# hustvl/ControlAR

Hardware: AMD Instinct MI355X
Metric: images/sec/GPU, LlamaGen-XL t2i canny 512x512 (1024 tok); 1/2/4/8-GPU scaling (higher is better)
Workload: dtype bf16

## Files before the change

### controlar_amd/csrc/gemm.hip

```cpp
#include "car_common.h"
#include "gemm_gather.h"
#include <cstdio>
#include <cstdlib>

__device__ __forceinline__ void ld8bf(const bf16_t* p, float (&v)[8]) {
    const uint4 u = *(const uint4*)p; const unsigned w[4] = {u.x, u.y, u.z, u.w};
#pragma unroll
    for (int e = 0; e < 4; ++e) { v[2 * e] = __uint_as_float(w[e] << 16); v[2 * e + 1] = __uint_as_float(w[e] & 0xffff0000u); }
}
enum { EP_VEC = 0, EP_SCALAR = 1, EP_SWIGLU = 2 };
__device__ __forceinline__ float gate_act(int kind, float a) { return kind == 2 ? gelu_tanh_f(a) : silu_f(a); }
__device__ __forceinline__ int strip_path(const GemmP& p, long zC, long zR) {
    if (p.swiglu) return EP_SWIGLU;
    const bool vec = (p.N & 7) == 0 && (p.ldc & 7) == 0 && (!p.R || (p.ldr & 7) == 0) && p.bias_mode != BIAS_M &&
                     ((zC | zR) & 7) == 0 && ((uintptr_t)p.C & 15) == 0 && (!p.R || ((uintptr_t)p.R & 15) == 0);
    return vec ? EP_VEC : EP_SCALAR;
}
template <int PATH>
__device__ __forceinline__ void store_strip(const GemmP& p, const float* strip, int mb, int nb, long zC, long zR, int lane) {
    const bf16_t* bias = (const bf16_t*)p.bias; const bf16_t* scale = (const bf16_t*)p.scale; const bf16_t* R = (const bf16_t*)p.R;
    if (PATH == EP_SWIGLU) {
        const int rr = lane >> 2, c = (lane & 3) * 8, src = (c >> 4) * 32 + (c & 15), m = mb + rr;
        if (m < p.M && nb + src + 24 <= p.N && (p.ldc & 7) == 0 && (zC & 7) == 0) {
            unsigned o[4];
// ... 220 lines not shown
        if (kt + 2 < nk) issue(buf >= 1 ? buf - 1 : G2_NS - 1);
#pragma unroll
        for (int kk = 0; kk < 2; ++kk) {
            bf16x8 a[4], b[4];
#pragma unroll
            for (int i = 0; i < 4; ++i) { const int r = wm * 64 + i * 16 + fr; a[i] = *(const bf16x8*)(S2A(buf) + r * G2_BK + (((kk * 4 + fq) ^ (r & 7)) << 3)); }
#pragma unroll
            for (int j = 0; j < 4; ++j) { const int r = wn * 64 + j * 16 + fr; b[j] = *(const bf16x8*)(S2B(buf) + r * G2_BK + (((kk * 4 + fq) ^ (r & 7)) << 3)); }
#pragma unroll
            for (int i = 0; i < 4; ++i)
#pragma unroll
                for (int j = 0; j < 4; ++j)
                    acc[i][j] = __builtin_amdgcn_mfma_f32_16x16x32_bf16(a[i], b[j], acc[i][j], 0, 0, 0);
        }
        buf = buf + 1 == G2_NS ? 0 : buf + 1;
    }
    __syncthreads();

    float* strip = (float*)smem2 + wave * (16 * 68);
    const int path = strip_path(p, zC, zR);
#define STRIP_LOOP(PATH)                                                                          \
    _Pragma("unroll") for (int i = 0; i < 4; ++i) {                                               \
        _Pragma("unroll") for (int j = 0; j < 4; ++j) {                                           \
            const f32x4 q = acc[i][j];                                                            \
            float* d = strip + ((lane >> 4) * 4) * 68 + j * 16 + fr;                              \
            d[0] = q[0]; d[68] = q[1]; d[136] = q[2]; d[204] = q[3];                              \
        }                                                                                         \
        __builtin_amdgcn_wave_barrier();                                                          \
        store_strip<PATH>(p, strip, m0 + wm * 64 + i * 16, n0 + wn * 64, zC, zR, lane);           \
        __builtin_amdgcn_wave_barrier();                                                          \
    }
    if (path == EP_VEC) { STRIP_LOOP(EP_VEC) } else if (path == EP_SWIGLU) { STRIP_LOOP(EP_SWIGLU) } else { STRIP_LOOP(EP_SCALAR) }
#undef STRIP_LOOP
}

#define CH_HALO_MAX (18 * 18)
template <int UPS>
__global__ __launch_bounds__(512) void conv3_halo_kernel(GemmP p) {
    extern __shared__ __attribute__((aligned(16))) bf16_t smem3[];
    constexpr int HD = (16 >> UPS) + 2, HP = HD * HD;
    bf16_t* halo = smem3;
    bf16_t* wst = smem3 + CH_HALO_MAX * 128;
    const int tid = threadIdx.x, lane = tid & 63, wave = tid >> 6;
    const int wm = wave >> 1, wn = wave & 1;
    const int n0 = blockIdx.x * BN, tile = blockIdx.y;
    const int tw = p.Wo >> 4, th = p.Ho >> 4;
    const int b = tile / (tw * th), t2 = tile - b * (tw * th), ty = t2 / tw, tx = t2 - ty * tw;
    const int Hin = p.Ho >> UPS, Win = p.Wo >> UPS;
    const int hy0 = ((16 * ty - 1) >> UPS), hx0 = ((16 * tx - 1) >> UPS);
    const bf16_t* A = (const bf16_t*)p.A + (long)b * Hin * Win * p.Cin;
    const bf16_t* W = (const bf16_t*)p.W;
    const bf16_t* zero = (const bf16_t*)p.zero;
    const int fr = lane & 15, fq = lane >> 4;
    const int lr = lane >> 3, gchunk = ((lane & 7) ^ lr) * 8;
    const bf16_t* wrow[2];
#pragma unroll
    for (int i = 0; i < 2; ++i) { const int r = i * 64 + wave * 8 + lr; wrow[i] = (n0 + r) < p.N ? W + (long)(n0 + r) * p.ldw + gchunk : nullptr; }
    auto issue_w = [&](int buf, int kglob) {
#pragma unroll
        for (int i = 0; i < 2; ++i) {
            const bf16_t* src = wrow[i] ? wrow[i] + kglob : zero;
            __builtin_amdgcn_global_load_lds((gptr_t*)src, (lptr_t*)(wst + buf * (BN * G2_BK) + (i * 64 + wave * 8) * G2_BK), 16, 0, 0);
        }
    };
    f32x4 acc[4][4];
#pragma unroll
    for (int i = 0; i < 4; ++i)
#pragma unroll
        for (int j = 0; j < 4; ++j) acc[i][j] = (f32x4){0.f, 0.f, 0.f, 0.f};
    const int nchunk = p.Cin >> 7;
    for (int ch = 0; ch < nchunk; ++ch) {
        __syncthreads();
        for (int q = wave; q * 4 < HP; q += 8) {
            const int pix = q * 4 + (lane >> 4), slot = lane & 15;
            const int hy = pix / HD, hx = pix - hy * HD, iy = hy0 + hy, ix = hx0 + hx;
            const bf16_t* src = zero;
            if (pix < HP && iy >= 0 && iy < Hin && ix >= 0 && ix < Win) src = A + ((long)iy * Win + ix) * p.Cin + ch * 128 + ((slot ^ (pix & 15)) << 3);
            __builtin_amdgcn_global_load_lds((gptr_t*)src, (lptr_t*)(halo + q * 4 * 128), 16, 0, 0);
        }
        auto kglob = [&](int s_) { return (s_ >> 1) * p.Cin + ch * 128 + (s_ & 1) * 64; };
        issue_w(0, kglob(0)); issue_w(1, kglob(1));
        int buf = 0;
        for (int s_ = 0; s_ < 18; ++s_) {
            if (s_ == 0) asm volatile("s_waitcnt vmcnt(2)" ::: "memory");
            else if (s_ + 1 < 18) asm volatile("s_waitcnt vmcnt(2)" ::: "memory");
            else asm volatile("s_waitcnt vmcnt(0)" ::: "memory");
            __builtin_amdgcn_s_barrier();
            if (s_ + 2 < 18) issue_w(buf >= 1 ? buf - 1 : 2, kglob(s_ + 2));
            const int tap = s_ >> 1, c64 = s_ & 1, dy = tap / 3 - 1, dx = tap % 3 - 1;
            const bf16_t* ws = wst + buf * (BN * G2_BK);
#pragma unroll
            for (int kk = 0; kk < 2; ++kk) {
                bf16x8 a[4], bb[4];
#pragma unroll
                for (int i = 0; i < 4; ++i) {
                    const int h = (((16 * ty + wm * 4 + i + dy) >> UPS) - hy0) * HD + (((16 * tx + fr + dx) >> UPS) - hx0);
                    a[i] = *(const bf16x8*)(halo + h * 128 + (((c64 * 8 + kk * 4 + fq) ^ (h & 15)) << 3));
                }
#pragma unroll
                for (int j = 0; j < 4; ++j) { const int r = wn * 64 + j * 16 + fr; bb[j] = *(const bf16x8*)(ws + r * G2_BK + (((kk * 4 + fq) ^ (r & 7)) << 3)); }
#pragma unroll
                for (int i = 0; i < 4; ++i)
#pragma unroll
                    for (int j = 0; j < 4; ++j)
                        acc[i][j] = __builtin_amdgcn_mfma_f32_16x16x32_bf16(a[i], bb[j], acc[i][j], 0, 0, 0);
            }
            buf = buf + 1 == 3 ? 0 : buf + 1;
        }
    }
    __syncthreads();
    const bf16_t* bias = (const bf16_t*)p.bias; const bf16_t* R = (const bf16_t*)p.R;
    float* strip = (float*)smem3 + wave * (16 * 68);
    const int ec = (lane & 7) * 8, en = n0 + wn * 64 + ec;
    float bv[8];
    {
        const uint4 u = p.bias_mode == BIAS_N ? *(const uint4*)(bias + en) : make_uint4(0, 0, 0, 0);
        const unsigned w[4] = {u.x, u.y, u.z, u.w};
#pragma unroll
        for (int e = 0; e < 4; ++e) { bv[2 * e] = __uint_as_float(w[e] << 16); bv[2 * e + 1] = __uint_as_float(w[e] & 0xffff0000u); }
    }
#pragma unroll
    for (int i = 0; i < 4; ++i) {
#pragma unroll
        for (int j = 0; j < 4; ++j) {
            const f32x4 q = acc[i][j];
            float* d = strip + ((lane >> 4) * 4) * 68 + j * 16 + fr;
            d[0] = q[0]; d[68] = q[1]; d[136] = q[2]; d[204] = q[3];
        }
        __builtin_amdgcn_wave_barrier();
        const int oy = 16 * ty + wm * 4 + i;
#pragma unroll
        for (int pass = 0; pass < 2; ++pass) {
            const int rr = pass * 8 + (lane >> 3);
            const long mr = ((long)b * p.Ho + oy) * p.Wo + 16 * tx + rr;
            const float4 s0 = *(const float4*)(strip + rr * 68 + ec), s1 = *(const float4*)(strip + rr * 68 + ec + 4);
            float v[8] = {s0.x, s0.y, s0.z, s0.w, s1.x, s1.y, s1.z, s1.w};
#pragma unroll
            for (int e = 0; e < 8; ++e) v[e] = bf2f(f2bf(v[e] + bv[e]));
            if (R) {
                const uint4 u = *(const uint4*)(R + mr * p.ldr + en);
                const unsigned w[4] = {u.x, u.y, u.z, u.w};
#pragma unroll
                for (int e = 0; e < 4; ++e) { v[2 * e] = v[2 * e] + __uint_as_float(w[e] << 16); v[2 * e + 1] = v[2 * e + 1] + __uint_as_float(w[e] & 0xffff0000u); }
            }
            uint4 o;
            o.x = (unsigned)f2bf(v[0]) | ((unsigned)f2bf(v[1]) << 16); o.y = (unsigned)f2bf(v[2]) | ((unsigned)f2bf(v[3]) << 16);
            o.z = (unsigned)f2bf(v[4]) | ((unsigned)f2bf(v[5]) << 16); o.w = (unsigned)f2bf(v[6]) | ((unsigned)f2bf(v[7]) << 16);
            *(uint4*)((bf16_t*)p.C + mr * p.ldc + en) = o;
        }
        __builtin_amdgcn_wave_barrier();
    }
}

#define CH64_HALO_PIX 328
template <int UPS, int GNP>
__global__ __launch_bounds__(512, 4) void conv3_halo64_kernel(GemmP p) {
    extern __shared__ __attribute__((aligned(16))) bf16_t smem4[];
    constexpr int HD = (16 >> UPS) + 2, HP = HD * HD;
    bf16_t* halo = smem4;
    bf16_t* wst = smem4 + CH64_HALO_PIX * 64;
    const int tid = threadIdx.x, lane = tid & 63, wave = tid >> 6;
    const int wm = wave >> 1, wn = wave & 1;
    const int n0 = blockIdx.x * BN, tile = blockIdx.y;
    const int tw = p.Wo >> 4, th = p.Ho >> 4;
    const int b = tile / (tw * th), t2 = tile - b * (tw * th), ty = t2 / tw, tx = t2 - ty * tw;
    const int Hin = p.Ho >> UPS, Win = p.Wo >> UPS;
    const int hy0 = ((16 * ty - 1) >> UPS), hx0 = ((16 * tx - 1) >> UPS);
    const bf16_t* A = (const bf16_t*)p.A + (long)b * Hin * Win * p.Cin;
    const bf16_t* W = (const bf16_t*)p.W;
    const bf16_t* zero = (const bf16_t*)p.zero;
    const int fr = lane & 15, fq = lane >> 4;
    const int lr = lane >> 3, gchunk = ((lane & 7) ^ lr) * 8;
    const bf16_t* wrow[2];
#pragma unroll
    for (int i = 0; i < 2; ++i) { const int r = i * 64 + wave * 8 + lr; wrow[i] = (n0 + r) < p.N ? W + (long)(n0 + r) * p.ldw + gchunk : nullptr; }
    auto issue_w = [&](int buf, int kglob) {
#pragma unroll
        for (int i = 0; i < 2; ++i) {
            const bf16_t* src = wrow[i] ? wrow[i] + kglob : zero;
            __builtin_amdgcn_global_load_lds((gptr_t*)src, (lptr_t*)(wst + buf * (BN * G2_BK) + (i * 64 + wave * 8) * G2_BK), 16, 0, 0);
        }
    };
    f32x4 acc[4][4];
#pragma unroll
    for (int i = 0; i < 4; ++i)
#pragma unroll
        for (int j = 0; j < 4; ++j) acc[i][j] = (f32x4){0.f, 0.f, 0.f, 0.f};
    const int ngrp = p.Cin >> 6;
    for (int cg = 0; cg < ngrp; ++cg) {
        __syncthreads();
        for (int q = wave; q * 8 < HP; q += 8) {
            const int pix = q * 8 + (lane >> 3), slot = lane & 7;
            const int hy = pix / HD, hx = pix - hy * HD, iy = hy0 + hy, ix = hx0 + hx;
            const bf16_t* src = zero;
            if (pix < HP && iy >= 0 && iy < Hin && ix >= 0 && ix < Win) src = A + ((long)iy * Win + ix) * p.Cin + cg * 64 + ((slot ^ (pix & 7)) << 3);
            __builtin_amdgcn_global_load_lds((gptr_t*)src, (lptr_t*)(halo + q * 8 * 64), 16, 0, 0);
        }
        issue_w(0, cg * 64);
        int buf = 0;
        for (int tap = 0; tap < 9; ++tap) {
            asm volatile("s_waitcnt vmcnt(0)" ::: "memory");
            __builtin_amdgcn_s_barrier();
            if (tap + 1 < 9) issue_w(buf ^ 1, (tap + 1) * p.Cin + cg * 64);
            const int dy = tap / 3 - 1, dx = tap % 3 - 1;
            const bf16_t* ws = wst + buf * (BN * G2_BK);
#pragma unroll
            for (int kk = 0; kk < 2; ++kk) {
                bf16x8 a[4], bb[4];
#pragma unroll
                for (int i = 0; i < 4; ++i) {
                    const int h = (((16 * ty + wm * 4 + i + dy) >> UPS) - hy0) * HD + (((16 * tx + fr + dx) >> UPS) - hx0);
                    a[i] = *(const bf16x8*)(halo + h * 64 + (((kk * 4 + fq) ^ (h & 7)) << 3));
                }
#pragma unroll
                for (int j = 0; j < 4; ++j) { const int r = wn * 64 + j * 16 + fr; bb[j] = *(const bf16x8*)(ws + r * G2_BK + (((kk * 4 + fq) ^ (r & 7)) << 3)); }
#pragma unroll
                for (int i = 0; i < 4; ++i)
#pragma unroll
                    for (int j = 0; j < 4; ++j)
                        acc[i][j] = __builtin_amdgcn_mfma_f32_16x16x32_bf16(a[i], bb[j], acc[i][j], 0, 0, 0);
            }
            buf ^= 1;
        }
    }
    __syncthreads();
    const bf16_t* bias = (const bf16_t*)p.bias; const bf16_t* R = (const bf16_t*)p.R;
    float* strip = (float*)smem4 + wave * (16 * 68);
    const int ec = (lane & 7) * 8, en = n0 + wn * 64 + ec;
    float bv[8];
    {
        const uint4 u = p.bias_mode == BIAS_N ? *(const uint4*)(bias + en) : make_uint4(0, 0, 0, 0);
        const unsigned w[4] = {u.x, u.y, u.z, u.w};
#pragma unroll
        for (int e = 0; e < 4; ++e) { bv[2 * e] = __uint_as_float(w[e] << 16); bv[2 * e + 1] = __uint_as_float(w[e] & 0xffff0000u); }
    }
    float gs[8], gq[8];
#pragma unroll
    for (int e = 0; e < 8; ++e) { gs[e] = 0.f; gq[e] = 0.f; }
#pragma unroll
    for (int i = 0; i < 4; ++i) {
#pragma unroll
        for (int j = 0; j < 4; ++j) {
            const f32x4 q = acc[i][j];
            float* d = strip + ((lane >> 4) * 4) * 68 + j * 16 + fr;
            d[0] = q[0]; d[68] = q[1]; d[136] = q[2]; d[204] = q[3];
        }
        __builtin_amdgcn_wave_barrier();
        const int oy = 16 * ty + wm * 4 + i;
#pragma unroll
        for (int pass = 0; pass < 2; ++pass) {
            const int rr = pass * 8 + (lane >> 3);
            const long mr = ((long)b * p.Ho + oy) * p.Wo + 16 * tx + rr;
            const float4 s0 = *(const float4*)(strip + rr * 68 + ec), s1 = *(const float4*)(strip + rr * 68 + ec + 4);
            float v[8] = {s0.x, s0.y, s0.z, s0.w, s1.x, s1.y, s1.z, s1.w};
#pragma unroll
            for (int e = 0; e < 8; ++e) v[e] = bf2f(f2bf(v[e] + bv[e]));
            if (R) {
                const uint4 u = *(const uint4*)(R + mr * p.ldr + en);
                const unsigned w[4] = {u.x, u.y, u.z, u.w};
#pragma unroll
                for (int e = 0; e < 4; ++e) { v[2 * e] = v[2 * e] + __uint_as_float(w[e] << 16); v[2 * e + 1] = v[2 * e + 1] + __uint_as_float(w[e] & 0xffff0000u); }
            }
            uint4 o;
            o.x = (unsigned)f2bf(v[0]) | ((unsigned)f2bf(v[1]) << 16); o.y = (unsigned)f2bf(v[2]) | ((unsigned)f2bf(v[3]) << 16);
            o.z = (unsigned)f2bf(v[4]) | ((unsigned)f2bf(v[5]) << 16); o.w = (unsigned)f2bf(v[6]) | ((unsigned)f2bf(v[7]) << 16);
            *(uint4*)((bf16_t*)p.C + mr * p.ldc + en) = o;
            if (GNP) {
#pragma unroll
                for (int e = 0; e < 8; ++e) { const float r_ = bf2f(f2bf(v[e])); gs[e] += r_; gq[e] += r_ * r_; }
            }
        }
        __builtin_amdgcn_wave_barrier();
    }
    if (GNP) {
        float* red = (float*)smem4 + 8 * (16 * 68);
#pragma unroll
        for (int e = 0; e < 8; ++e) {
#pragma unroll
            for (int o_ = 8; o_ < 64; o_ <<= 1) { gs[e] += __shfl_xor(gs[e], o_, 64); gq[e] += __shfl_xor(gq[e], o_, 64); }
        }
        if (lane < 8) {
#pragma unroll
            for (int e = 0; e < 8; ++e) { red[(wave * 64 + lane * 8 + e) * 2] = gs[e]; red[(wave * 64 + lane * 8 + e) * 2 + 1] = gq[e]; }
        }
        __syncthreads();
        if (tid < 128) {
            const int wn2 = tid >> 6, cc = tid & 63;
            float s_ = 0.f, q_ = 0.f;
#pragma unroll
            for (int w4 = 0; w4 < 4; ++w4) { const float* r2 = red + ((w4 * 2 + wn2) * 64 + cc) * 2; s_ += r2[0]; q_ += r2[1]; }
            if (n0 + tid < p.N) {
                float* o2 = p.gn_part + ((long)b * (tw * th) + t2) * 2 * p.N;
                o2[n0 + tid] = s_; o2[p.N + n0 + tid] = q_;
            }
        }
    }
}

template <int AMODE>
__global__ __launch_bounds__(256) void gemm_f32_kernel(GemmP p) {
    __shared__ __attribute__((aligned(16))) float sA[2][16][68];
    __shared__ __attribute__((aligned(16))) float sB[2][16][68];
    const int tid = threadIdx.x, tx = tid & 15, ty = tid >> 4;
    const int z = blockIdx.z, z0 = z / p.nb1, z1 = z - z0 * p.nb1;
    const float* A = (const float*)p.A + z0 * p.sA0 + z1 * p.sA1;
    const float* W = (const float*)p.W + z0 * p.sW0 + z1 * p.sW1;
    const long zC = z0 * p.sC0 + z1 * p.sC1, zR = z0 * p.sR0 + z1 * p.sR1;
    const int m0 = blockIdx.y * 64, n0 = blockIdx.x * 64;
    const int lrow = tid >> 2, lkc = (tid & 3) * 4;
    const Geo geo = { p.M, p.Cin, p.Ho, p.Wo, p.ups, p.lda, p.patch };
    const ARow ar = make_arow<AMODE>(geo, m0 + lrow);
    const bool wok = (n0 + lrow) < p.N;
    const float* wp = W + (long)(n0 + lrow) * p.ldw + lkc;
    float4 ra, rb;
    const float4 zero4 = make_float4(0, 0, 0, 0);
    auto gload = [&](int kt) {
        long o = a_off<AMODE>(geo, ar, kt * 16 + lkc);
        ra = zero4; rb = zero4;
        if (o >= 0) ra = *(const float4*)(A + o);
        if (wok) rb = *(const float4*)(wp + (long)kt * 16);
    };
    auto sstore = [&](int buf) {
        sA[buf][lkc + 0][lrow] = ra.x; sA[buf][lkc + 1][lrow] = ra.y; sA[buf][lkc + 2][lrow] = ra.z; sA[buf][lkc + 3][lrow] = ra.w;
        sB[buf][lkc + 0][lrow] = rb.x; sB[buf][lkc + 1][lrow] = rb.y; sB[buf][lkc + 2][lrow] = rb.z; sB[buf][lkc + 3][lrow] = rb.w;
    };
    float acc[4][4] = {};
    const int nk = p.K / 16;
    gload(0); sstore(0);
    __syncthreads();
    for (int kt = 0; kt < nk; ++kt) {
        const int buf = kt & 1;
        if (kt + 1 < nk) gload(kt + 1);
#pragma unroll
        for (int k = 0; k < 16; ++k) {
            const float4 a = *(const float4*)&sA[buf][k][ty * 4];
            const float4 b = *(const float4*)&sB[buf][k][tx * 4];
            const float av[4] = {a.x, a.y, a.z, a.w}, bv[4] = {b.x, b.y, b.z, b.w};
#pragma unroll
            for (int i = 0; i < 4; ++i)
#pragma unroll
                for (int j = 0; j < 4; ++j) acc[i][j] = fmaf(av[i], bv[j], acc[i][j]);
        }
        if (kt + 1 < nk) sstore(buf ^ 1);
        __syncthreads();
    }
    const float* bias = (const float*)p.bias; const float* scale = (const float*)p.scale; const float* R = (const float*)p.R;
#pragma unroll
    for (int i = 0; i < 4; ++i)
#pragma unroll
        for (int j = 0; j < 4; ++j) {
            const int m = m0 + ty * 4 + i, n = n0 + tx * 4 + j;
            if (m < p.M && n < p.N)
                ((float*)p.C)[zC + (long)m * p.ldc + n] = epi_value<float>(p, bias, scale, R, zR, m, (long)m, n, acc[i][j]);
        }
}

typedef __attribute__((ext_vector_type(4))) float f4_t;
#define F32_LD 20
template <int AMODE>
__global__ __launch_bounds__(256) void gemm_f32_mfma_kernel(GemmP p) {
    __shared__ __attribute__((aligned(16))) float sA[2][128 * F32_LD];
    __shared__ __attribute__((aligned(16))) float sB[2][128 * F32_LD];
    const int tid = threadIdx.x, lane = tid & 63, wave = tid >> 6, q4 = lane >> 4, c16 = lane & 15;
    const int wm = wave >> 1, wn = wave & 1;
    const int z = blockIdx.z, z0 = z / p.nb1, z1 = z - z0 * p.nb1;
    const float* A = (const float*)p.A + z0 * p.sA0 + z1 * p.sA1;
    const float* W = (const float*)p.W + z0 * p.sW0 + z1 * p.sW1;
    const long zC = z0 * p.sC0 + z1 * p.sC1, zR = z0 * p.sR0 + z1 * p.sR1;
    const int m0 = blockIdx.y * 128, n0 = blockIdx.x * 128;
    const int lrow = tid >> 1, lkc = (tid & 1) * 8;
    const Geo geo = { p.M, p.Cin, p.Ho, p.Wo, p.ups, p.lda, p.patch };
    const ARow ar = make_arow<AMODE>(geo, m0 + lrow);
    const bool wok = (n0 + lrow) < p.N;
    const float* wp = W + (long)(n0 + lrow) * p.ldw + lkc;
    float4 ra[2], rb[2];
    const float4 zero4 = make_float4(0, 0, 0, 0);
    auto gload = [&](int kt) {
#pragma unroll
        for (int c = 0; c < 2; ++c) {
            const long o = a_off<AMODE>(geo, ar, kt * 16 + lkc + c * 4);
            ra[c] = zero4; rb[c] = zero4;
            if (o >= 0) ra[c] = *(const float4*)(A + o);
            if (wok) rb[c] = *(const float4*)(wp + (long)kt * 16 + c * 4);
        }
    };
    auto sstore = [&](int buf) {
#pragma unroll
        for (int c = 0; c < 2; ++c) { *(float4*)&sA[buf][lrow * F32_LD + lkc + c * 4] = ra[c]; *(float4*)&sB[buf][lrow * F32_LD + lkc + c * 4] = rb[c]; }
    };
    f4_t acc[4][4];
#pragma unroll
    for (int i = 0; i < 4; ++i)
#pragma unroll
        for (int j = 0; j < 4; ++j) acc[i][j] = (f4_t){0.f, 0.f, 0.f, 0.f};
    const int nk = p.K / 16;
    gload(0); sstore(0);
    __syncthreads();
    for (int kt = 0; kt < nk; ++kt) {
        const int buf = kt & 1;
        if (kt + 1 < nk) gload(kt + 1);
        f4_t xa[4], wa[4];
#pragma unroll
        for (int j = 0; j < 4; ++j) xa[j] = *(const f4_t*)&sA[buf][(wm * 64 + j * 16 + c16) * F32_LD + q4 * 4];
#pragma unroll
        for (int i = 0; i < 4; ++i) wa[i] = *(const f4_t*)&sB[buf][(wn * 64 + i * 16 + c16) * F32_LD + q4 * 4];
#pragma unroll
        for (int s = 0; s < 4; ++s)
#pragma unroll
            for (int i = 0; i < 4; ++i)
#pragma unroll
                for (int j = 0; j < 4; ++j) acc[i][j] = __builtin_amdgcn_mfma_f32_16x16x4f32(wa[i][s], xa[j][s], acc[i][j], 0, 0, 0);
        if (kt + 1 < nk) sstore(buf ^ 1);
        __syncthreads();
    }
    const float* bias = (const float*)p.bias; const float* scale = (const float*)p.scale; const float* R = (const float*)p.R;
    const bool vec = (p.ldc & 3) == 0 && ((zC & 3) == 0) && (((uintptr_t)p.C & 15) == 0);
#pragma unroll
    for (int j = 0; j < 4; ++j) {
        const int m = m0 + wm * 64 + j * 16 + c16;
        if (m >= p.M) continue;
#pragma unroll
        for (int i = 0; i < 4; ++i) {
            const int n = n0 + wn * 64 + i * 16 + q4 * 4;
            if (n >= p.N) continue;
            float v[4];
#pragma unroll
            for (int r = 0; r < 4; ++r) v[r] = (n + r < p.N) ? epi_value<float>(p, bias, scale, R, zR, m, (long)m, n + r, acc[i][j][r]) : 0.f;
            float* dst = (float*)p.C + zC + (long)m * p.ldc + n;
            if (vec && n + 3 < p.N) *(float4*)dst = make_float4(v[0], v[1], v[2], v[3]);
            else { for (int r = 0; r < 4; ++r) if (n + r < p.N) dst[r] = v[r]; }
        }
    }
}

static void* g_zero_page[16] = {};
static void* zero_page_for(int dev) {
    if (dev < 0 || dev >= 16) return nullptr;
    if (!g_zero_page[dev]) { if (hipMalloc(&g_zero_page[dev], 256) == hipSuccess) (void)hipMemset(g_zero_page[dev], 0, 256); else { g_zero_page[dev] = nullptr; (void)hipGetLastError(); } }
    return g_zero_page[dev];
}
static bool conv3_halo_plan(int mode, int amode, const GemmP& p, int* dev_out, void** zero_out) {
    int dev = 0; (void)hipGetDevice(&dev);
    if (dev_out) *dev_out = dev;
    if (!(mode == 1 && amode == AMODE_CONV3 && p.Cin % 128 == 0 && (p.Ho & 15) == 0 && (p.Wo & 15) == 0 && (p.ups == 0 || p.ups == 1) && p.K == 9 * p.Cin && p.ldw % 8 == 0 &&
          (uintptr_t)p.A % 16 == 0 && (uintptr_t)p.W % 16 == 0 && !p.swiglu && !p.out_f32 && p.act == ACT_NONE && (p.nb0 <= 1) && (p.nb1 <= 1) && p.alpha == 1.0f &&
          p.N % 128 == 0 && !p.scale && p.bias_mode != BIAS_M && p.ldc % 8 == 0 && (!p.R || p.ldr % 8 == 0) && !CAR_KNOB("CAR_GEMM_V1") && !CAR_KNOB("CAR_NO_HALO"))) return false;
    void* z = zero_page_for(dev);
    if (zero_out) *zero_out = z;
    return z != nullptr;
}
extern "C" int car_conv3_halo64_ok(int mode, const GemmP* pp) {
    return conv3_halo_plan(mode, AMODE_CONV3, *pp, nullptr, nullptr) && !CAR_KNOB("CAR_CONV_HALO128") && !CAR_KNOB("CAR_GN_UNFUSED");
}
extern "C" int car_gemm_split_ok(int amode, const GemmP* pp);
extern "C" hipError_t car_launch_gemm_split(int amode, const GemmP* pp, hipStream_t st);
extern "C" int car_gemm_route(int mode, int amode, const GemmP* pp) {
    const GemmP& p = *pp;
    const int nb0 = p.nb0 <= 0 ? 1 : p.nb0, nb1 = p.nb1 <= 0 ? 1 : p.nb1;
    if (mode == 1) {
        if (conv3_halo_plan(mode, amode, p, nullptr, nullptr)) {
            const bool halo128 = CAR_KNOB("CAR_CONV_HALO128") != nullptr;
            if (p.gn_part && (halo128 || CAR_KNOB("CAR_GN_UNFUSED"))) return CAR_ROUTE_REFUSE_GN;
            return halo128 ? CAR_ROUTE_HALO128 : CAR_ROUTE_HALO64;
        }
        if (p.gn_part) return CAR_ROUTE_REFUSE_GN;
        if (p.K % BKK != 0) return CAR_ROUTE_REFUSE_K;
        const bool al16 = ((uintptr_t)p.A % 16 == 0) && ((uintptr_t)p.W % 16 == 0) && p.ldw % 8 == 0 && p.sW0 % 8 == 0 && p.sW1 % 8 == 0 && p.sA0 % 8 == 0 && p.sA1 % 8 == 0;
        const long tiles = (long)((p.N + BN - 1) / BN) * ((p.M + G2_BM - 1) / G2_BM) * nb0 * nb1;
        int dev = 0; (void)hipGetDevice(&dev);
        const bool ok2 = dev >= 0 && dev < 16 && p.K % G2_BK == 0 && p.K >= 512 && al16 && tiles >= 512 && !CAR_KNOB("CAR_GEMM_V1") &&
                         (amode == AMODE_PLAIN ? p.lda % 8 == 0 : (amode == AMODE_CONV3 && p.Cin % G2_BK == 0));
        return ok2 ? CAR_ROUTE_BF16_GLDS : CAR_ROUTE_BF16_REG;
    }
    if (p.gn_part) return CAR_ROUTE_REFUSE_GN;
    if (p.K % 16 != 0) return CAR_ROUTE_REFUSE_K;
    if (p.split3 && car_gemm_split_ok(amode, &p)) return CAR_ROUTE_F32_SPLIT;
    const bool mfma_ok = p.ldw % 4 == 0 && ((uintptr_t)p.A & 15) == 0 && ((uintptr_t)p.W & 15) == 0 && p.sA0 % 4 == 0 && p.sA1 % 4 == 0 && p.sW0 % 4 == 0 && p.sW1 % 4 == 0 &&
                         (amode == AMODE_PLAIN ? p.lda % 4 == 0 : p.Cin % 4 == 0);
    return mfma_ok ? CAR_ROUTE_F32_MFMA : CAR_ROUTE_F32_VALU;
}
extern "C" int car_launch_gemm(int mode, int amode, const GemmP* pp, hipStream_t st) {
    GemmP p = *pp;
    if (p.nb0 <= 0) p.nb0 = 1;
    if (p.nb1 <= 0) p.nb1 = 1;
    const int route = car_gemm_route(mode, amode, &p);
    if (route < 0) {
        if (route == CAR_ROUTE_REFUSE_K) fprintf(stderr, "car_launch_gemm: K = %d is not a multiple of %d (%s kernels): refused, nothing launched\n", p.K, mode == 1 ? BKK : 16, mode == 1 ? "bf16" : "fp32");
        return route;
    }
    static bool attr_set[16] = {}, attr3[16] = {}, attr4[16] = {};
    int dev = 0; (void)hipGetDevice(&dev);
    if (mode == 1) { if (amode != AMODE_CONV3 || (p.Ho & 15) || (p.Wo & 15) || CAR_KNOB("CAR_CONV_LINEAR")) p.patch = 0; }
    else p.patch = 0;
    switch (route) {
    case CAR_ROUTE_HALO64: {
        p.zero = zero_page_for(dev);
        const dim3 g3((p.N + BN - 1) / BN, (unsigned)((long)p.M / 256));
        const size_t sh4 = (size_t)(CH64_HALO_PIX * 64 + 2 * BN * G2_BK) * 2;
        if (!attr4[dev]) {
            (void)hipFuncSetAttribute((const void*)conv3_halo64_kernel<0, 0>, hipFuncAttributeMaxDynamicSharedMemorySize, (int)sh4);
            (void)hipFuncSetAttribute((const void*)conv3_halo64_kernel<1, 0>, hipFuncAttributeMaxDynamicSharedMemorySize, (int)sh4);
            (void)hipFuncSetAttribute((const void*)conv3_halo64_kernel<0, 1>, hipFuncAttributeMaxDynamicSharedMemorySize, (int)sh4);
            (void)hipFuncSetAttribute((const void*)conv3_halo64_kernel<1, 1>, hipFuncAttributeMaxDynamicSharedMemorySize, (int)sh4);
            attr4[dev] = true;
        }
        if (p.ups == 0) { if (p.gn_part) hipLaunchKernelGGL((conv3_halo64_kernel<0, 1>), g3, dim3(512), sh4, st, p); else hipLaunchKernelGGL((conv3_halo64_kernel<0, 0>), g3, dim3(512), sh4, st, p); }
        else { if (p.gn_part) hipLaunchKernelGGL((conv3_halo64_kernel<1, 1>), g3, dim3(512), sh4, st, p); else hipLaunchKernelGGL((conv3_halo64_kernel<1, 0>), g3, dim3(512), sh4, st, p); }
        return 0;
    }
    case CAR_ROUTE_HALO128: {
        p.zero = zero_page_for(dev);
        const dim3 g3((p.N + BN - 1) / BN, (unsigned)((long)p.M / 256));
        const size_t sh3 = (size_t)(CH_HALO_MAX * 128 + 3 * BN * G2_BK) * 2;
        if (!attr3[dev]) {
            (void)hipFuncSetAttribute((const void*)conv3_halo_kernel<0>, hipFuncAttributeMaxDynamicSharedMemorySize, (int)sh3);
            (void)hipFuncSetAttribute((const void*)conv3_halo_kernel<1>, hipFuncAttributeMaxDynamicSharedMemorySize, (int)sh3);
            attr3[dev] = true;
        }
        if (p.ups == 0) hipLaunchKernelGGL(conv3_halo_kernel<0>, g3, dim3(512), sh3, st, p);
        else hipLaunchKernelGGL(conv3_halo_kernel<1>, g3, dim3(512), sh3, st, p);
        return 0;
    }
    case CAR_ROUTE_BF16_GLDS: {
        const size_t sh = (size_t)G2_NS * G2_STAGE * 2;
        if (!attr_set[dev]) {
            (void)hipFuncSetAttribute((const void*)gemm_bf16_glds_kernel<AMODE_PLAIN>, hipFuncAttributeMaxDynamicSharedMemorySize, (int)sh);
            (void)hipFuncSetAttribute((const void*)gemm_bf16_glds_kernel<AMODE_CONV3>, hipFuncAttributeMaxDynamicSharedMemorySize, (int)sh);
            attr_set[dev] = true;
        }
        if ((p.zero = zero_page_for(dev)) != nullptr) {
            dim3 g2((p.N + BN - 1) / BN, (p.M + G2_BM - 1) / G2_BM, p.nb0 * p.nb1);
            if (amode == AMODE_PLAIN) hipLaunchKernelGGL(gemm_bf16_glds_kernel<AMODE_PLAIN>, g2, dim3(512), sh, st, p);
            else hipLaunchKernelGGL(gemm_bf16_glds_kernel<AMODE_CONV3>, g2, dim3(512), sh, st, p);
            return 0;
        }
        [[fallthrough]];
    }
    case CAR_ROUTE_BF16_REG: {
        dim3 g((p.N + BN - 1) / BN, (p.M + BM - 1) / BM, p.nb0 * p.nb1);
        if (amode == AMODE_PLAIN) hipLaunchKernelGGL(gemm_bf16_kernel<AMODE_PLAIN>, g, dim3(256), 0, st, p);
        else if (amode == AMODE_CONV3S2) hipLaunchKernelGGL(gemm_bf16_kernel<AMODE_CONV3S2>, g, dim3(256), 0, st, p);
        else hipLaunchKernelGGL(gemm_bf16_kernel<AMODE_CONV3>, g, dim3(256), 0, st, p);
        return 0;
    }
    case CAR_ROUTE_F32_SPLIT:
        return car_launch_gemm_split(amode, &p, st) == hipSuccess ? 0 : -2;
    case CAR_ROUTE_F32_MFMA: {
        dim3 g((p.N + 127) / 128, (p.M + 127) / 128, p.nb0 * p.nb1);
        if (amode == AMODE_PLAIN) hipLaunchKernelGGL(gemm_f32_mfma_kernel<AMODE_PLAIN>, g, dim3(256), 0, st, p);
        else if (amode == AMODE_CONV3S2) hipLaunchKernelGGL(gemm_f32_mfma_kernel<AMODE_CONV3S2>, g, dim3(256), 0, st, p);
        else hipLaunchKernelGGL(gemm_f32_mfma_kernel<AMODE_CONV3>, g, dim3(256), 0, st, p);
        return 0;
    }
    default: {
        dim3 g((p.N + 63) / 64, (p.M + 63) / 64, p.nb0 * p.nb1);
        if (amode == AMODE_PLAIN) hipLaunchKernelGGL(gemm_f32_kernel<AMODE_PLAIN>, g, dim3(256), 0, st, p);
        else if (amode == AMODE_CONV3S2) hipLaunchKernelGGL(gemm_f32_kernel<AMODE_CONV3S2>, g, dim3(256), 0, st, p);
        else hipLaunchKernelGGL(gemm_f32_kernel<AMODE_CONV3>, g, dim3(256), 0, st, p);
        return 0;
    }
    }
}
```

Measured before the change: 44.85.

## Fully unroll halo64 conv tap loop with hand-scheduled LDS reads and waits

Adds a new default path in the 64-channel halo conv kernel. It unrolls all 9 taps at compile time, uses precomputed LDS byte offsets with inline ds_read_b128 immediates, and staggers the A/B fragment loads with fine-grained lgkmcnt waits and sched barriers so LDS reads overlap the MFMAs. The halo swizzle now uses the column index, which lets the address math be hoisted out of the loop, and the wave index is made uniform via readfirstlane. The old loop stays available behind a knob, and a bit-exact A/B check harness is added. The hand-written waitcnt logic and schedule are fragile and could raise register pressure at 4 waves per SIMD.

```diff
diff --git a/controlar_amd/csrc/gemm.hip b/controlar_amd/csrc/gemm.hip
--- a/controlar_amd/csrc/gemm.hip
+++ b/controlar_amd/csrc/gemm.hip
@@ -396,14 +396,27 @@
     }
 }
 
+template <int I> struct car_ic { static constexpr int value = I; };
+template <int N, int I = 0, class F> __device__ __forceinline__ void car_static_for(F&& f) { if constexpr (I < N) { f(car_ic<I>{}); car_static_for<N, I + 1>(f); } }
+template <int UPS> constexpr int h64_a_off(int tap, int g) { const int i = g & 3, dy = tap / 3 - 1; return (UPS ? (i + dy + 2) >> 1 : i + dy + 1) * ((16 >> UPS) + 2) * 128; }
+constexpr int h64_b_off(int buf, int j) { return buf * (BN * G2_BK * 2) + j * (16 * G2_BK * 2); }
+template <int OFF> __device__ __forceinline__ void lds_read16(bf16x8& v, unsigned addr) { asm volatile("ds_read_b128 %0, %1 offset:%2" : "=v"(v) : "v"(addr), "n"(OFF) : "memory"); }
+template <int N> __device__ __forceinline__ void lds_wait(bf16x8& x0) { asm volatile("s_waitcnt lgkmcnt(%1)" : "+v"(x0) : "n"(N)); }
+template <int N> __device__ __forceinline__ void lds_wait(bf16x8& x0, bf16x8& x1) { asm volatile("s_waitcnt lgkmcnt(%2)" : "+v"(x0), "+v"(x1) : "n"(N)); }
+template <int N> __device__ __forceinline__ void lds_wait(bf16x8& x0, bf16x8& x1, bf16x8& x2) { asm volatile("s_waitcnt lgkmcnt(%3)" : "+v"(x0), "+v"(x1), "+v"(x2) : "n"(N)); }
+template <int N> __device__ __forceinline__ void lds_wait(bf16x8& x0, bf16x8& x1, bf16x8& x2, bf16x8& x3, bf16x8& x4, bf16x8& x5) {
+    asm volatile("s_waitcnt lgkmcnt(%6)" : "+v"(x0), "+v"(x1), "+v"(x2), "+v"(x3), "+v"(x4), "+v"(x5) : "n"(N));
+}
 #define CH64_HALO_PIX 328
-template <int UPS, int GNP>
+template <int UPS, int GNP, int V1>
 __global__ __launch_bounds__(512, 4) void conv3_halo64_kernel(GemmP p) {
     extern __shared__ __attribute__((aligned(16))) bf16_t smem4[];
     constexpr int HD = (16 >> UPS) + 2, HP = HD * HD;
     bf16_t* halo = smem4;
     bf16_t* wst = smem4 + CH64_HALO_PIX * 64;
-    const int tid = threadIdx.x, lane = tid & 63, wave = tid >> 6;
+    const int tid = threadIdx.x, lane = tid & 63;
+    const int wave = V1 ? tid >> 6 : __builtin_amdgcn_readfirstlane(tid >> 6);
+
     const int wm = wave >> 1, wn = wave & 1;
     const int n0 = blockIdx.x * BN, tile = blockIdx.y;
     const int tw = p.Wo >> 4, th = p.Ho >> 4;
@@ -430,6 +443,10 @@
     for (int i = 0; i < 4; ++i)
 #pragma unroll
         for (int j = 0; j < 4; ++j) acc[i][j] = (f32x4){0.f, 0.f, 0.f, 0.f};
+    unsigned ho[3];
+#pragma unroll
+    for (int d = 0; d < 3; ++d) { const int col = UPS ? (fr + d + 1) >> 1 : fr + d; ho[d] = (unsigned)((wm * (4 >> UPS) * HD + col) * 128 + ((fq ^ (col & 7)) << 4)); }
+    const unsigned wo = (unsigned)(CH64_HALO_PIX * 128 + (wn * 64 + fr) * 128 + ((fq ^ (fr & 7)) << 4));
     const int ngrp = p.Cin >> 6;
     for (int cg = 0; cg < ngrp; ++cg) {
         __syncthreads();
@@ -437,10 +454,45 @@
             const int pix = q * 8 + (lane >> 3), slot = lane & 7;
             const int hy = pix / HD, hx = pix - hy * HD, iy = hy0 + hy, ix = hx0 + hx;
             const bf16_t* src = zero;
-            if (pix < HP && iy >= 0 && iy < Hin && ix >= 0 && ix < Win) src = A + ((long)iy * Win + ix) * p.Cin + cg * 64 + ((slot ^ (pix & 7)) << 3);
+            if (pix < HP && iy >= 0 && iy < Hin && ix >= 0 && ix < Win) src = A + ((long)iy * Win + ix) * p.Cin + cg * 64 + ((slot ^ ((V1 ? pix : hx) & 7)) << 3);
             __builtin_amdgcn_global_load_lds((gptr_t*)src, (lptr_t*)(halo + q * 8 * 64), 16, 0, 0);
         }
         issue_w(0, cg * 64);
+        if constexpr (!V1) {
+            bf16x8 a[3], b0[4], b1[4];
+            car_static_for<9>([&](auto tap_) {
+                constexpr int tap = decltype(tap_)::value, buf = tap & 1, last = tap == 8;
+                asm volatile("s_waitcnt vmcnt(0)" ::: "memory");
+                __builtin_amdgcn_s_barrier();
+                if (tap + 1 < 9) issue_w(buf ^ 1, (tap + 1) * p.Cin + cg * 64);
+                if (tap == 0) { lds_read16<h64_a_off<UPS>(0, 0)>(a[0], ho[0]); lds_read16<h64_a_off<UPS>(0, 1)>(a[1], ho[0]); }
+                car_static_for<4>([&](auto j_) { constexpr int j = decltype(j_)::value; lds_read16<h64_b_off(buf, j)>(b0[j], wo); });
+                car_static_for<8>([&](auto g_) {
+                    constexpr int g = decltype(g_)::value, G = tap * 8 + g, i = g & 3, c = G % 3, n2 = (G + 2) % 3;
+                    if constexpr (g + 2 < 8) lds_read16<h64_a_off<UPS>(tap, g + 2)>(a[n2], ho[tap % 3] ^ (unsigned)(((g + 2) >> 2) << 6));
+                    else if constexpr (!last) lds_read16<h64_a_off<UPS>(tap + 1, g - 6)>(a[n2], ho[(tap + 1) % 3]);
+                    if constexpr (g == 1) lds_read16<h64_b_off(buf, 0)>(b1[0], wo ^ 64u);
+                    if constexpr (g == 2) lds_read16<h64_b_off(buf, 1)>(b1[1], wo ^ 64u);
+                    if constexpr (g == 0) lds_wait<1>(a[c], a[(G + 1) % 3], b0[0], b0[1], b0[2], b0[3]);
+                    if constexpr (g == 2 || g == 3) lds_wait<4>(a[c]);
+                    if constexpr (g == 4) lds_wait<4>(a[c], b1[0], b1[1]);
+                    if constexpr (g == 6) lds_wait<last ? 1 : 2>(a[c]);
+                    if constexpr (g == 7) lds_wait<last ? 0 : 2>(a[c]);
+                    car_static_for<4>([&](auto j_) {
+                        constexpr int j = decltype(j_)::value;
+                        if constexpr (g == 4 && j == 2) { __builtin_amdgcn_sched_barrier(0); lds_wait<2>(a[(G + 1) % 3], b1[2]); }
+                        if constexpr (g == 4 && j == 3) { __builtin_amdgcn_sched_barrier(0); lds_wait<1>(b1[3]); }
+                        acc[i][j] = __builtin_amdgcn_mfma_f32_16x16x32_bf16(a[c], g < 4 ? b0[j] : b1[j], acc[i][j], 0, 0, 0);
+                        if constexpr (g == 3 && j < 2) {
+                            __builtin_amdgcn_sched_barrier(0);
+                            lds_read16<h64_b_off(buf, 2 + j)>(b1[2 + j], wo ^ 64u);
+                        }
+                    });
+                    __builtin_amdgcn_sched_barrier(0);
+                });
+            });
+            continue;
+        }
         int buf = 0;
         for (int tap = 0; tap < 9; ++tap) {
             asm volatile("s_waitcnt vmcnt(0)" ::: "memory");
@@ -741,15 +793,15 @@
         p.zero = zero_page_for(dev);
         const dim3 g3((p.N + BN - 1) / BN, (unsigned)((long)p.M / 256));
         const size_t sh4 = (size_t)(CH64_HALO_PIX * 64 + 2 * BN * G2_BK) * 2;
+        typedef void (*halo64_fn)(GemmP);
+        static const halo64_fn fn4[2][2][2] = {{{conv3_halo64_kernel<0, 0, 0>, conv3_halo64_kernel<0, 1, 0>}, {conv3_halo64_kernel<1, 0, 0>, conv3_halo64_kernel<1, 1, 0>}},
+                                               {{conv3_halo64_kernel<0, 0, 1>, conv3_halo64_kernel<0, 1, 1>}, {conv3_halo64_kernel<1, 0, 1>, conv3_halo64_kernel<1, 1, 1>}}};
         if (!attr4[dev]) {
-            (void)hipFuncSetAttribute((const void*)conv3_halo64_kernel<0, 0>, hipFuncAttributeMaxDynamicSharedMemorySize, (int)sh4);
-            (void)hipFuncSetAttribute((const void*)conv3_halo64_kernel<1, 0>, hipFuncAttributeMaxDynamicSharedMemorySize, (int)sh4);
-            (void)hipFuncSetAttribute((const void*)conv3_halo64_kernel<0, 1>, hipFuncAttributeMaxDynamicSharedMemorySize, (int)sh4);
-            (void)hipFuncSetAttribute((const void*)conv3_halo64_kernel<1, 1>, hipFuncAttributeMaxDynamicSharedMemorySize, (int)sh4);
+            for (int i = 0; i < 8; ++i) (void)hipFuncSetAttribute((const void*)fn4[i >> 2][(i >> 1) & 1][i & 1], hipFuncAttributeMaxDynamicSharedMemorySize, (int)sh4);
             attr4[dev] = true;
         }
-        if (p.ups == 0) { if (p.gn_part) hipLaunchKernelGGL((conv3_halo64_kernel<0, 1>), g3, dim3(512), sh4, st, p); else hipLaunchKernelGGL((conv3_halo64_kernel<0, 0>), g3, dim3(512), sh4, st, p); }
-        else { if (p.gn_part) hipLaunchKernelGGL((conv3_halo64_kernel<1, 1>), g3, dim3(512), sh4, st, p); else hipLaunchKernelGGL((conv3_halo64_kernel<1, 0>), g3, dim3(512), sh4, st, p); }
+        const int v1 = CAR_KNOB("CAR_CONV_TAPLOOP_V1") != nullptr;
+        hipLaunchKernelGGL(fn4[v1][p.ups][p.gn_part != nullptr], g3, dim3(512), sh4, st, p);
         return 0;
     }
     case CAR_ROUTE_HALO128: {
diff --git a/experiments/conv_pipe_check.hip b/experiments/conv_pipe_check.hip
--- /dev/null
+++ b/experiments/conv_pipe_check.hip
@@ -0,0 +1,186 @@
+#ifndef CAR_DEV_KNOBS
+#error "conv_pipe_check needs -DCAR_DEV_KNOBS: without it CAR_KNOB() is a null constant, CAR_CONV_TAPLOOP_V1 selects nothing and the new loop would be compared with itself"
+#endif
+#include "../controlar_amd/csrc/gemm.hip"
+#include "../controlar_amd/csrc/gemm_split.hip"
+#include "../controlar_amd/csrc/ops.hip"
+
+#include <cmath>
+#include <cstdio>
+#include <cstdlib>
+#include <cstring>
+#include <vector>
+
+extern "C" { int g_car_knob_hits = 0; }
+
+#define CK(x) do { hipError_t e_ = (x); if (e_ != hipSuccess) { printf("HIP error %s at %s:%d\n", hipGetErrorString(e_), __FILE__, __LINE__); exit(2); } } while (0)
+static const char* const SWITCH = "CAR_CONV_TAPLOOP_V1";
+static const size_t GUARD = 512;
+static int g_fail = 0;
+
+static unsigned hsh(unsigned a, unsigned b, unsigned seed) {
+    unsigned x = a * 2654435761u + b * 0x85ebca6bu + seed * 0x9e3779b9u; x ^= x >> 15; x *= 2246822519u; x ^= x >> 13; x *= 3266489917u; x ^= x >> 16; return x;
+}
+static bf16_t rnd_bf16(unsigned i, unsigned seed, unsigned expo) { const unsigned x = hsh(i, 0u, seed); return (bf16_t)((x & 0x807fu) | ((((x >> 7) & 3u) + expo) << 7)); }
+
+struct Case { const char* name; int B, Ho, Wo, Cin, Cout, ups; bool bias, resid, gn; };
+
+struct Bufs {
+    bf16_t *x = nullptr, *w = nullptr, *bias = nullptr, *r = nullptr, *y = nullptr; float* part = nullptr;
+    size_t nin = 0, nw = 0, nout = 0, npart = 0;
+};
+static void alloc(const Case& c, Bufs& d) {
+    const int Hin = c.Ho >> c.ups, Win = c.Wo >> c.ups;
+    d.nin = (size_t)c.B * Hin * Win * c.Cin; d.nw = (size_t)c.Cout * 9 * c.Cin; d.nout = (size_t)c.B * c.Ho * c.Wo * c.Cout;
+    d.npart = (size_t)c.B * (c.Ho / 16) * (c.Wo / 16) * 2 * c.Cout;
+    CK(hipMalloc(&d.x, d.nin * 2)); CK(hipMalloc(&d.w, d.nw * 2)); CK(hipMalloc(&d.bias, (size_t)c.Cout * 2)); CK(hipMalloc(&d.r, d.nout * 2));
+    CK(hipMalloc(&d.y, (d.nout + 2 * GUARD) * 2)); CK(hipMalloc(&d.part, (d.npart + 2 * GUARD) * 4));
+}
+static void release(Bufs& d) { for (void* q : {(void*)d.x, (void*)d.w, (void*)d.bias, (void*)d.r, (void*)d.y, (void*)d.part}) CK(hipFree(q)); }
+static void up(bf16_t* dst, const std::vector<bf16_t>& h) { CK(hipMemcpy(dst, h.data(), h.size() * 2, hipMemcpyHostToDevice)); }
+
+static void launch(const Case& c, const Bufs& d, bool v1, std::vector<unsigned char>& out, std::vector<unsigned char>& part) {
+    CK(hipMemset(d.y, 0xff, (d.nout + 2 * GUARD) * 2)); CK(hipMemset(d.part, 0xff, (d.npart + 2 * GUARD) * 4));
+    GemmP p; memset(&p, 0, sizeof(p));
+    p.A = d.x; p.W = d.w; p.C = d.y + GUARD; p.ldw = 9L * c.Cin; p.ldc = c.Cout; p.M = c.B * c.Ho * c.Wo; p.N = c.Cout; p.K = 9 * c.Cin; p.alpha = 1.f; p.nb0 = p.nb1 = 1;
+    p.Ho = c.Ho; p.Wo = c.Wo; p.Cin = c.Cin; p.ups = c.ups; p.patch = 1;
+    if (c.bias) { p.bias = d.bias; p.bias_mode = BIAS_N; }
+    if (c.resid) { p.R = d.r; p.ldr = c.Cout; }
+    if (v1) setenv(SWITCH, "1", 1); else unsetenv(SWITCH);
+    if (c.gn) { if (!car_conv3_halo64_ok(1, &p)) { printf("FAIL %s: not eligible for the halo route\n", c.name); exit(3); } p.gn_part = d.part + GUARD; }
+    const int route = car_gemm_route(1, AMODE_CONV3, &p);
+    if (route != CAR_ROUTE_HALO64) { printf("FAIL %s: route %d, expected HALO64\n", c.name, route); exit(3); }
+    if (car_launch_gemm(1, AMODE_CONV3, &p, 0) != 0) { printf("FAIL %s: launch refused\n", c.name); exit(3); }
+    unsetenv(SWITCH);
+    CK(hipDeviceSynchronize()); CK(hipGetLastError());
+    out.resize((d.nout + 2 * GUARD) * 2); part.resize((d.npart + 2 * GUARD) * 4);
+    CK(hipMemcpy(out.data(), d.y, out.size(), hipMemcpyDeviceToHost)); CK(hipMemcpy(part.data(), d.part, part.size(), hipMemcpyDeviceToHost));
+}
+static bool guards_intact(const std::vector<unsigned char>& b, size_t guard_bytes) {
+    for (size_t i = 0; i < guard_bytes; ++i) if (b[i] != 0xff || b[b.size() - 1 - i] != 0xff) return false;
+    return true;
+}
+
+static void run_ab(const Case& c) {
+    Bufs d; alloc(c, d);
+    std::vector<bf16_t> hx(d.nin), hw(d.nw), hb(c.Cout), hr(d.nout);
+    for (size_t i = 0; i < d.nin; ++i) hx[i] = rnd_bf16((unsigned)i, 11u, 124u);
+    for (size_t i = 0; i < d.nw; ++i) hw[i] = rnd_bf16((unsigned)i, 12u, 119u);
+    for (int i = 0; i < c.Cout; ++i) hb[i] = rnd_bf16((unsigned)i, 13u, 122u);
+    for (size_t i = 0; i < d.nout; ++i) hr[i] = rnd_bf16((unsigned)i, 14u, 124u);
+    up(d.x, hx); up(d.w, hw); up(d.bias, hb); up(d.r, hr);
+    std::vector<unsigned char> o0, p0, o1, p1;
+    launch(c, d, false, o0, p0); launch(c, d, true, o1, p1);
+    const bool same_out = o0 == o1, same_part = p0 == p1, g = guards_intact(o0, GUARD * 2) && guards_intact(p0, GUARD * 4);
+    bool written = false; for (size_t i = GUARD * 2; i < GUARD * 2 + d.nout * 2 && !written; i += 2) written = !(o0[i] == 0xff && o0[i + 1] == 0xff);
+    bool part_ok = true;
+    if (!c.gn) for (size_t i = 0; i < d.npart * 4; ++i) if (p0[GUARD * 4 + i] != 0xff) part_ok = false;
+    const bool ok = same_out && same_part && g && written && part_ok;
+    printf("%s  new vs round-3 loop  %-52s out %s, partials %s, guards %s\n", ok ? "ok  " : "FAIL", c.name, same_out ? "equal" : "BITS DIFFER", same_part ? "equal" : "BITS DIFFER", g ? "intact" : "BROKEN");
+    if (!ok) ++g_fail;
+    release(d);
+}
+
+struct Exact { std::vector<bf16_t> x, w, b; std::vector<int> y; std::vector<long> ps, pq; int max_mag = 0; };
+static int xa(unsigned pix, int ch) {
+    const int blk = ch >> 7;
+    if ((ch & 127) != (int)(hsh(pix, (unsigned)blk, 21u) & 127u)) return 0;
+    const unsigned h = hsh(pix, (unsigned)ch, 22u); const int m = 1 + (int)(h & 1u); return (h & 0x100u) ? -m : m;
+}
+static int xw(int n, int k) { return (int)(hsh((unsigned)n, (unsigned)k, 23u) % 5u) - 2; }
+static int xb(int n) { return (int)(hsh((unsigned)n, 0u, 24u) % 17u) - 8; }
+static void build_exact(const Case& c, Exact& e) {
+    const int Hin = c.Ho >> c.ups, Win = c.Wo >> c.ups, K = 9 * c.Cin;
+    e.x.resize((size_t)Hin * Win * c.Cin); e.w.resize((size_t)c.Cout * K); e.b.resize(c.Cout); e.y.assign((size_t)c.Ho * c.Wo * c.Cout, 0);
+    for (int pix = 0; pix < Hin * Win; ++pix) for (int ch = 0; ch < c.Cin; ++ch) e.x[(size_t)pix * c.Cin + ch] = f2bf((float)xa((unsigned)pix, ch));
+    for (int n = 0; n < c.Cout; ++n) for (int k = 0; k < K; ++k) e.w[(size_t)n * K + k] = f2bf((float)xw(n, k));
+    for (int n = 0; n < c.Cout; ++n) e.b[n] = f2bf((float)xb(n));
+    e.ps.assign(c.Cout, 0); e.pq.assign(c.Cout, 0);
+    for (int oy = 0; oy < c.Ho; ++oy) for (int ox = 0; ox < c.Wo; ++ox) for (int n = 0; n < c.Cout; ++n) {
+        int sum = xb(n), mag = std::abs(xb(n));
+        for (int tap = 0; tap < 9; ++tap) {
+            const int uy = oy + tap / 3 - 1, ux = ox + tap % 3 - 1;
+            if (uy < 0 || uy >= c.Ho || ux < 0 || ux >= c.Wo) continue;
+            const unsigned pix = (unsigned)((uy >> c.ups) * Win + (ux >> c.ups));
+            for (int blk = 0; blk < c.Cin / 128; ++blk) {
+                const int ch = blk * 128 + (int)(hsh(pix, (unsigned)blk, 21u) & 127u), a = xa(pix, ch), w = xw(n, tap * c.Cin + ch);
+                sum += a * w; mag += std::abs(a * w);
+            }
+        }
+        if (mag > e.max_mag) e.max_mag = mag;
+        e.y[((size_t)oy * c.Wo + ox) * c.Cout + n] = sum; e.ps[n] += sum; e.pq[n] += (long)sum * sum;
+    }
+}
+static bool exact_precondition(const Exact& e) { return e.max_mag <= 256; }
+static void run_exact(const Case& c) {
+    Exact e; build_exact(c, e);
+    if (!exact_precondition(e)) { printf("FAIL %s: sum of magnitudes %d > 256, the reference is not exact\n", c.name, e.max_mag); ++g_fail; return; }
+    Bufs d; alloc(c, d);
+    up(d.x, e.x); up(d.w, e.w); up(d.bias, e.b);
+    std::vector<unsigned char> want_o((d.nout + 2 * GUARD) * 2, 0xff), want_p((d.npart + 2 * GUARD) * 4, 0xff);
+    for (size_t i = 0; i < d.nout; ++i) { const bf16_t v = f2bf((float)e.y[i]); memcpy(&want_o[(GUARD + i) * 2], &v, 2); }
+    for (int n = 0; n < c.Cout; ++n) { const float s = (float)e.ps[n], q = (float)e.pq[n]; memcpy(&want_p[(GUARD + n) * 4], &s, 4); memcpy(&want_p[(GUARD + c.Cout + n) * 4], &q, 4); }
+    for (int v1 = 0; v1 < 2; ++v1) {
+        std::vector<unsigned char> o, pp; launch(c, d, v1 != 0, o, pp);
+        const bool so = o == want_o, sp = pp == want_p;
+        printf("%s  exact integers       %-40s %-12s out %s, partials %s (max sum of magnitudes %d)\n", so && sp ? "ok  " : "FAIL", c.name, v1 ? "round-3 loop" : "new loop", so ? "equal" : "BITS DIFFER", sp ? "equal" : "BITS DIFFER", e.max_mag);
+        if (!(so && sp)) ++g_fail;
+    }
+    release(d);
+}
+
+static void run_time(const Case& c) {
+    Bufs d; alloc(c, d);
+    std::vector<bf16_t> h(std::max(std::max(d.nin, d.nw), d.nout));
+    for (size_t i = 0; i < h.size(); ++i) h[i] = rnd_bf16((unsigned)i, 31u, 120u);
+    CK(hipMemcpy(d.x, h.data(), d.nin * 2, hipMemcpyHostToDevice)); CK(hipMemcpy(d.w, h.data(), d.nw * 2, hipMemcpyHostToDevice));
+    CK(hipMemcpy(d.bias, h.data(), (size_t)c.Cout * 2, hipMemcpyHostToDevice)); CK(hipMemcpy(d.r, h.data(), d.nout * 2, hipMemcpyHostToDevice));
+    GemmP p; memset(&p, 0, sizeof(p));
+    p.A = d.x; p.W = d.w; p.C = d.y + GUARD; p.ldw = 9L * c.Cin; p.ldc = c.Cout; p.M = c.B * c.Ho * c.Wo; p.N = c.Cout; p.K = 9 * c.Cin; p.alpha = 1.f; p.nb0 = p.nb1 = 1;
+    p.Ho = c.Ho; p.Wo = c.Wo; p.Cin = c.Cin; p.ups = c.ups; p.patch = 1; p.bias = d.bias; p.bias_mode = BIAS_N; p.R = d.r; p.ldr = c.Cout; p.gn_part = c.gn ? d.part + GUARD : nullptr;
+    hipEvent_t t0, t1; CK(hipEventCreate(&t0)); CK(hipEventCreate(&t1));
+    float us[2][3];
+    for (int round = 0; round < 3; ++round) for (int v1 = 0; v1 < 2; ++v1) {
+        if (v1) setenv(SWITCH, "1", 1); else unsetenv(SWITCH);
+        for (int i = 0; i < 2; ++i) if (car_launch_gemm(1, AMODE_CONV3, &p, 0) != 0) { printf("launch refused\n"); exit(3); }
+        CK(hipDeviceSynchronize()); CK(hipEventRecord(t0, 0));
+        for (int i = 0; i < 6; ++i) car_launch_gemm(1, AMODE_CONV3, &p, 0);
+        CK(hipEventRecord(t1, 0)); CK(hipEventSynchronize(t1)); CK(hipGetLastError());
+        float ms; CK(hipEventElapsedTime(&ms, t0, t1)); us[v1][round] = ms * 1e3f / 6;
+    }
+    unsetenv(SWITCH);
+    const double fl = 2.0 * c.B * c.Ho * c.Wo * (double)c.Cout * 9 * c.Cin;
+    auto mn = [](const float* v) { return std::min(v[0], std::min(v[1], v[2])); }; auto mx = [](const float* v) { return std::max(v[0], std::max(v[1], v[2])); };
+    printf("%-30s gn=%d  new %8.1f %8.1f %8.1f us (%4.0f TFLOP/s)   round-3 %8.1f %8.1f %8.1f us (%4.0f TFLOP/s)   x%.3f  %s\n", c.name, (int)c.gn, us[0][0], us[0][1], us[0][2], fl / mn(us[0]) / 1e6,
+           us[1][0], us[1][1], us[1][2], fl / mn(us[1]) / 1e6, mn(us[1]) / mn(us[0]), mx(us[0]) < mn(us[1]) ? "ranges apart, new faster" : mx(us[1]) < mn(us[0]) ? "ranges apart, new SLOWER" : "ranges overlap");
+    fflush(stdout);
+    release(d);
+}
+
+int main(int argc, char** argv) {
+    const char* mode = argc > 1 ? argv[1] : "quick";
+    unsetenv(SWITCH);
+    for (const char* k : {"CAR_CONV_HALO128", "CAR_GEMM_V1", "CAR_NO_HALO", "CAR_CONV_LINEAR", "CAR_GN_UNFUSED"}) unsetenv(k);
+    const Case exact[] = {{"1 x 16x16 512->128 ups 0 bias + gn_part", 1, 16, 16, 512, 128, 0, true, false, true}, {"1 x 16x16 512->128 ups 1 bias + gn_part", 1, 16, 16, 512, 128, 1, true, false, true}};
+    if (!strcmp(mode, "selftest")) {
+        for (const Case& c : exact) { Exact e; build_exact(c, e); printf("%s  %s: max sum of magnitudes %d (bound 256)\n", exact_precondition(e) ? "ok  " : "FAIL", c.name, e.max_mag); if (!exact_precondition(e)) ++g_fail; }
+    } else if (!strcmp(mode, "time")) {
+        const Case times[] = {{"level 512^2 128->128", 24, 512, 512, 128, 128, 0, true, true, true}, {"upsample -> 512^2 128->128", 24, 512, 512, 128, 128, 1, true, false, true},
+                              {"level 256^2 256->128", 24, 256, 256, 256, 128, 0, true, false, true}, {"level 256^2 128->128", 24, 256, 256, 128, 128, 0, true, true, true},
+                              {"upsample -> 256^2 256->256", 24, 256, 256, 256, 256, 1, true, false, true}, {"level 128^2 256->256", 24, 128, 128, 256, 256, 0, true, true, true},
+                              {"level 64^2 512->512", 24, 64, 64, 512, 512, 0, true, true, true}, {"level 32^2 512->512", 24, 32, 32, 512, 512, 0, true, true, true},
+                              {"level 512^2 128->128", 24, 512, 512, 128, 128, 0, true, true, false}, {"upsample -> 512^2 128->128", 24, 512, 512, 128, 128, 1, true, false, false}};
+        for (const Case& c : times) run_time(c);
+    } else {
+        const Case ab[] = {{"1 x 16x16 128->128 ups 0, bias + R + gn_part", 1, 16, 16, 128, 128, 0, true, true, true},
+                           {"1 x 16x16 512->512 ups 0, gn_part", 1, 16, 16, 512, 512, 0, false, false, true},
+                           {"2 x 48x32 256->256 ups 1, bias + R", 2, 48, 32, 256, 256, 1, true, true, false},
+                           {"2 x 32x48 128->128 ups 0, no bias, no gn_part", 2, 32, 48, 128, 128, 0, false, false, false},
+                           {"1 x 32x32 384->128 ups 1, gn_part", 1, 32, 32, 384, 128, 1, false, false, true}};
+        for (const Case& c : ab) run_ab(c);
+        for (const Case& c : exact) run_exact(c);
+    }
+    if (g_fail) { printf("%d check(s) FAILED\n", g_fail); return 1; }
+    printf("all checks passed\n");
+    return 0;
+}
```

After: 44.97 (median of 6 runs). Within noise of the previous version (+0.3%).
